# tongdaxu/VQ-VAE-from-Gaussian-VAE

Measured on AMD Instinct MI355X. Metric: images/sec encode+quantize+decode, 256x256, codebook 2^16, higher is better.
Workload: dtype f32

## Files before the change

### vq-vae-from-gaussian-vae_amd/csrc/gq_conv3.h

```cpp
#pragma once
#include <type_traits>

#include "gq_common.h"
#include "gq_epilogue.h"
#include "gq_stats.h"
#include "gq_wino_gemm.h"

namespace gqhip {

constexpr int kC3TH = 8, kC3TW = 32;
constexpr int kC3PH = kC3TH + 2, kC3PW = kC3TW + 2;
constexpr int kC3Pix = kC3PH * kC3PW;
constexpr int kC3RS = 48;
constexpr int kC3Plane = kC3PH * kC3RS * 32;
constexpr int kC3Buf = 2 * kC3Plane;
constexpr int kC3Pieces = kC3Pix * 4;
constexpr int kC3Loads = (kC3Pieces + 255) / 256;

__device__ __forceinline__ int conv3_lds_off(int R, int x, int half) {
  return (R * kC3RS + x) * 32 + 16 * (half ^ ((x >> 3) & 1));
}

struct Conv3Params {
  const _Float16 *Xs;
  const _Float16 *Wf;
  const float *bias;
  const float *res;
  float *y;
  int64_t *stats;
  int H, W, nch, cpg;
  int cout, nnb;
  int tiles_x, tiles_y;
  long ntiles;
  long tiles_per_xcd;
  float mscale;
};

struct Conv3Tile {
  long b;
  int y0, x0, nb;
};
__device__ __forceinline__ bool conv3_tile(const Conv3Params &p, Conv3Tile &t, long vb = blockIdx.x) {
  const long k = vb >> 3;
  t.nb = (int)(k % p.nnb);
  const long tile = (long)(vb & 7) * p.tiles_per_xcd + k / p.nnb;
  if (tile >= p.ntiles) return false;
  const int tx = (int)(tile % p.tiles_x);
  const long t2 = tile / p.tiles_x;
  t.b = t2 / p.tiles_y;
  t.y0 = (int)(t2 % p.tiles_y) * kC3TH;
  t.x0 = tx * kC3TW;
  return true;
}

__device__ __forceinline__ void conv3_tap(const unsigned char *A, int dy, const f16x8 (&bq)[4], f32x16 (&acc)[4][2]) {
#pragma unroll
  for (int rr = 0; rr < 4; ++rr) {
#if defined(GQHIP_ABL) && (GQHIP_ABL & 256)
    const f16x8 ah = *reinterpret_cast<const f16x8 *>(A + dy * kC3RS * 32);
    const f16x8 al = ah;
#else
    const f16x8 ah = *reinterpret_cast<const f16x8 *>(A + (rr + dy) * kC3RS * 32);
    const f16x8 al = *reinterpret_cast<const f16x8 *>(A + (rr + dy) * kC3RS * 32 + kC3Plane);
#endif
#pragma unroll
    for (int j = 0; j < 2; ++j) {
      acc[rr][j] = __builtin_amdgcn_mfma_f32_32x32x16_f16(ah, bq[2 * j], acc[rr][j], 0, 0, 0);
      acc[rr][j] = __builtin_amdgcn_mfma_f32_32x32x16_f16(ah, bq[2 * j + 1], acc[rr][j], 0, 0, 0);
      acc[rr][j] = __builtin_amdgcn_mfma_f32_32x32x16_f16(al, bq[2 * j], acc[rr][j], 0, 0, 0);
    }
  }
}

template <int COUT, int RR>
__device__ __forceinline__ void conv3_epilogue(const Conv3Params &p, const Conv3Tile &t, const f32x16 (&acc)[RR][2], unsigned char *sA,
                                               int64_t *red, int wave, int wm, int wn) {
  constexpr int cout = COUT;
  const int lane = __lane_id(), tid = wave * 64 + lane;
  const int n = wn * 64 + 4 * (lane & 15);
  float *stage = reinterpret_cast<float *>(sA + wave * kEpiWaveBytes);
  f32x4 pb = {0.f, 0.f, 0.f, 0.f};
  if (p.bias) {
#pragma unroll
    for (int e = 0; e < 4; ++e) pb[e] = p.bias[t.nb * 128 + n + e];
  }
  const long o = ((t.b * p.H + t.y0 + RR * wm) * p.W + t.x0 + (lane >> 4)) * cout + t.nb * 128 + n;
  const long slice = (long)p.W * cout;
  StatPartial st;
  if (!p.stats) {
    if (p.res) epi_store<3, false>(acc, stage, lane, p.y, p.res, o, slice, 4 * cout, p.mscale, pb, st);
    else epi_store<2, false>(acc, stage, lane, p.y, nullptr, o, slice, 4 * cout, p.mscale, pb, st);
    return;
  }
  if constexpr (RR == 4) {
    if (p.res) epi_store<3, true>(acc, stage, lane, p.y, p.res, o, slice, 4 * cout, p.mscale, pb, st);
    else epi_store<2, true>(acc, stage, lane, p.y, nullptr, o, slice, 4 * cout, p.mscale, pb, st);
    stat_partial_flush(red + kStatWords * (n / p.cpg), st);
  } else {
    __shared__ double part[2 * 64 * 4];
    double *mine = part + (wn * 64 + lane) * 4;
    if (wm == 0) {
      if (p.res) epi_store<3, true>(acc, stage, lane, p.y, p.res, o, slice, 4 * cout, p.mscale, pb, st);
      else epi_store<2, true>(acc, stage, lane, p.y, nullptr, o, slice, 4 * cout, p.mscale, pb, st);
      mine[0] = st.v0; mine[1] = st.s; mine[2] = st.ss; mine[3] = (double)st.n;
    }
    __syncthreads();
    if (wm == 1) {
      st.v0 = mine[0]; st.s = mine[1]; st.ss = mine[2]; st.n = (int)mine[3];
      if (p.res) epi_store<3, true>(acc, stage, lane, p.y, p.res, o, slice, 4 * cout, p.mscale, pb, st);
      else epi_store<2, true>(acc, stage, lane, p.y, nullptr, o, slice, 4 * cout, p.mscale, pb, st);
      stat_partial_flush(red + kStatWords * (n / p.cpg), st);
    }
  }
  __syncthreads();
  const int gpb = 128 / p.cpg, groups = cout / p.cpg;
  if (tid < kStatWords * gpb) stat_flush_word(p.stats + kStatWords * (t.b * groups + t.nb * gpb) + tid, red[tid]);
}

#define GQ_C3_ZERO_ACC(acc)                                                                                         \
  _Pragma("unroll") for (int rr = 0; rr < 4; ++rr) _Pragma("unroll") for (int j = 0; j < 2; ++j) acc[rr][j] =       \
      f32x16{0.f, 0.f, 0.f, 0.f, 0.f, 0.f, 0.f, 0.f, 0.f, 0.f, 0.f, 0.f, 0.f, 0.f, 0.f, 0.f}

struct Conv3GnParams {
  Conv3Params c;
  const float *x;
  const float *gamma, *beta, *pre_bias;
  const int64_t *stats_in;
  int cin, cpg_in;
  double eps;
  float scale;
};

#ifndef GQHIP_C3_VALU_PER_MFMA
#define GQHIP_C3_VALU_PER_MFMA 3
#endif
#ifdef GQHIP_CLOCK_STAMPS
__device__ unsigned long long g_c3_stamps[4 * 8192];
#endif
template <int SILU, int COUT>
__global__ __launch_bounds__(256, 2) void conv3x3_gn_f16x3_kernel(const Conv3GnParams pp) {
  typedef _Float16 f16x4 __attribute__((ext_vector_type(4)));
  const Conv3Params &p = pp.c;
  __shared__ __attribute__((aligned(16))) unsigned char sA[2 * kC3Buf];
  __shared__ int64_t red[kStatWords * 32];
  __shared__ __attribute__((aligned(16))) float sAff[2][512];
  const int tid = threadIdx.x, lane = tid & 63, wave = __builtin_amdgcn_readfirstlane(tid >> 6);
  const int c = lane & 31, h = lane >> 5, wm = wave >> 1, wn = wave & 1;
#ifdef GQHIP_CLOCK_STAMPS
  const unsigned long long st_r0 = __builtin_amdgcn_s_memrealtime();
#endif
  Conv3Tile t;
  if (!conv3_tile(p, t)) return;
  const int H = p.H, W = p.W, cin = pp.cin;
  red[tid] = 0;
  {
    const int groups = cin / pp.cpg_in;
    const double n = (double)pp.cpg_in * (double)H * (double)W;
    for (int ch = tid; ch < cin; ch += 256) {
      const GnAffine f = gn_channel(gn_group(pp.stats_in + kStatWords * (t.b * groups + ch / pp.cpg_in), n, pp.eps), pp.gamma, pp.beta, pp.pre_bias, ch);
      sAff[0][ch] = f.a;
      sAff[1][ch] = f.sh;
    }
  }
  const int w = tid & 3, qs = tid >> 2;
  int goff[kC3Loads];
  unsigned inb = 0;
#pragma unroll
  for (int i = 0; i < kC3Loads; ++i) {
    int q = qs + 64 * i;
    q = q < kC3Pix ? q : kC3Pix - 1;
    const int R = q / kC3PW, px = q % kC3PW;
    const int gy = t.y0 - 1 + R, gx = t.x0 - 1 + px;
    const bool in = gy >= 0 && gy < H && gx >= 0 && gx < W;
    const int cy = clamp_index(gy, H), cx = clamp_index(gx, W);
    goff[i] = (cy * W + cx) * cin + 4 * w;
    inb |= (unsigned)(in ? 1 : 0) << i;
  }
  const float *xb = pp.x + t.b * (long)H * W * cin;
  f32x4 st[3];
  auto issue = [&](int i, int chunk) { st[i % 3] = *reinterpret_cast<const f32x4 *>(xb + goff[i] + chunk * 16); };
  auto convert = [&](int i, int chunk, int buf) {
    const int q = qs + 64 * i < kC3Pix ? qs + 64 * i : kC3Pix - 1;
    const f32x4 a4 = *reinterpret_cast<const f32x4 *>(&sAff[0][chunk * 16 + 4 * w]);
    const f32x4 sh4 = *reinterpret_cast<const f32x4 *>(&sAff[1][chunk * 16 + 4 * w]);
    const f32x4 v = gn_act<SILU>(st[i % 3], a4, sh4) * (((inb >> i) & 1) ? pp.scale : 0.f);
    f16x4 hi, lo;
#pragma unroll
    for (int e = 0; e < 4; ++e) {
      hi[e] = (_Float16)v[e];
      lo[e] = (_Float16)(v[e] - (float)hi[e]);
    }
    const int off = buf * kC3Buf + conv3_lds_off(q / kC3PW, q % kC3PW, w >> 1) + 8 * (w & 1);
    *reinterpret_cast<f16x4 *>(&sA[off]) = hi;
    *reinterpret_cast<f16x4 *>(&sA[off + kC3Plane]) = lo;
  };

  f32x16 acc[4][2];
  GQ_C3_ZERO_ACC(acc);
  int aoff[3];
#pragma unroll
  for (int dx = 0; dx < 3; ++dx) aoff[dx] = conv3_lds_off(4 * wm, c + dx, h);
  const unsigned char *wbase = reinterpret_cast<const unsigned char *>(p.Wf) + (4 * t.nb + 2 * wn) * 128 * 16;
  const int wl = lane * 16;
  const long wstep = (long)p.nnb * (512 * 16);
  f16x8 bs[3][4];
  auto load_b = [&](int ks, f16x8 (&dst)[4]) {
    const unsigned char *s = wbase + ks * wstep;
#pragma unroll
    for (int k = 0; k < 4; ++k) dst[k] = *reinterpret_cast<const f16x8 *>(s + k * 1024 + wl);
  };
  const int nks = p.nch * 9;
  load_b(0, bs[0]);
  load_b(1, bs[1]);
  __syncthreads();
  for (int i0 = 0; i0 < kC3Loads; i0 += 3) {
#pragma unroll
    for (int i = 0; i < 3; ++i) issue(i0 + i, 0);
#pragma unroll
    for (int i = 0; i < 3; ++i) convert(i0 + i, 0, 0);
  }
  __syncthreads();

#ifdef GQHIP_CLOCK_STAMPS
  const unsigned long long st_r1 = __builtin_amdgcn_s_memrealtime();
#endif
  auto run_chunk = [&](int chunk, auto more_tag) {
    constexpr bool more = decltype(more_tag)::value;
    const unsigned char *A = sA + (chunk & 1) * kC3Buf;
    const int nbuf = (chunk + 1) & 1;
#pragma unroll
    for (int tap = 0; tap < 9; ++tap) {
      const int ks = chunk * 9 + tap;
#if !(defined(GQHIP_ABL) && (GQHIP_ABL & 128))
      load_b(ks + 2 < nks ? ks + 2 : nks - 1, bs[(tap + 2) % 3]);
#endif
      conv3_tap(A + aoff[tap % 3], tap / 3, bs[tap % 3], acc);
#if !(defined(GQHIP_ABL) && (GQHIP_ABL & 64))
      if constexpr (more) {
        if (tap >= 3) convert(tap - 3, chunk + 1, nbuf);
        if (tap < kC3Loads) issue(tap, chunk + 1);
#if GQHIP_C3_VALU_PER_MFMA > 0
        if (tap >= 3) {
#pragma unroll
          for (int m = 0; m < 24; ++m) {
            __builtin_amdgcn_sched_group_barrier(0x008, 1, 0);
            __builtin_amdgcn_sched_group_barrier(0x002, GQHIP_C3_VALU_PER_MFMA, 0);
          }
        }
#endif
      }
#endif
      __builtin_amdgcn_sched_barrier(0);
    }
    __syncthreads();
  };
  for (int chunk = 0; chunk + 1 < p.nch; ++chunk) run_chunk(chunk, std::true_type{});
  run_chunk(p.nch - 1, std::false_type{});
#ifdef GQHIP_CLOCK_STAMPS
  const unsigned long long st_r2 = __builtin_amdgcn_s_memrealtime();
#endif
#if defined(GQHIP_ABL) && (GQHIP_ABL & 512)
  if (acc[0][0][0] == 12345.678f)
#endif
  conv3_epilogue<COUT>(p, t, acc, sA, red, wave, wm, wn);
#ifdef GQHIP_CLOCK_STAMPS
  if (tid == 0 && blockIdx.x < 8192) {
    unsigned long long *o = g_c3_stamps + 4 * blockIdx.x;
    o[0] = st_r0;
    o[1] = __builtin_amdgcn_s_memrealtime();
    o[2] = ((st_r1 - st_r0) << 32) | (st_r2 - st_r0);
    o[3] = ((unsigned long long)__builtin_amdgcn_s_getreg((31 << 11) | 20) << 32) | (unsigned)__builtin_amdgcn_s_getreg((31 << 11) | 4);
  }
#endif
}



struct Conv1Params {
  Conv3Params c;
  const float *x;
  const float *pre_bias;
  const float *scales_dev;
  float scale;
  int cin;
  const float *gamma, *beta;
  const int64_t *stats_in;
  int cpg_in;
  double eps;
  _Float16 *Q3, *K3, *V3;
  float sq, sv;
};

template <int COUT, int RR, int GN, int SPLIT>
__global__ __launch_bounds__(256, 2) void conv1x1_f16x3_kernel(const Conv1Params pp) {
  typedef _Float16 f16x4 __attribute__((ext_vector_type(4)));
  static_assert(RR == 4 || RR == 2, "rows of 32 pixels per wave");
  static_assert((SPLIT != 0) == (COUT == 0), "the split epilogue takes cout at run time");
  Conv3Params p = pp.c;
  constexpr int NI = 2 * RR;
  constexpr int kPlane = 32 * NI * 32, kChunk = 2 * kPlane, kStage = 2 * kChunk;
  static_assert(2 * kStage >= 4 * kEpiWaveBytes, "the epilogue stages through sA");
  __shared__ __attribute__((aligned(16))) unsigned char sA[2 * kStage];
  __shared__ int64_t red[kStatWords * 32];
  __shared__ __attribute__((aligned(16))) float sAff[2][GN ? 512 : 4];
  const int tid = threadIdx.x, lane = tid & 63, wave = __builtin_amdgcn_readfirstlane(tid >> 6);
  const int c = lane & 31, h = lane >> 5, wm = wave >> 1, wn = wave & 1;
  Conv3Tile t;
  if (!conv3_tile(p, t)) return;
  t.y0 = t.y0 / kC3TH * NI;
  red[tid] = 0;
  const float scale = pp.scales_dev ? pp.scales_dev[0] : pp.scale;
  if (pp.scales_dev) p.mscale = pp.scales_dev[1];
  const int cin = pp.cin, nst = cin / 32;
  if constexpr (GN != 0) {
    const int groups = cin / pp.cpg_in;
    const double n = (double)pp.cpg_in * (double)p.H * 32.0;
    for (int ch = tid; ch < cin; ch += 256) {
      const GnAffine f = gn_channel(gn_group(pp.stats_in + kStatWords * (t.b * groups + ch / pp.cpg_in), n, pp.eps), pp.gamma, pp.beta, pp.pre_bias, ch);
      sAff[0][ch] = f.a;
      sAff[1][ch] = f.sh;
    }
  }
  const int w8 = tid & 7, r0 = tid >> 3;
  const float *xb = pp.x + ((t.b * p.H + t.y0) * 32L + r0) * cin + 4 * w8;
  const float *pbp = (GN == 0 && pp.pre_bias) ? pp.pre_bias + 4 * w8 : nullptr;
  f32x4 pb4 = {0.f, 0.f, 0.f, 0.f}, a4 = pb4, sh4 = pb4;
  const int loff = (w8 >> 2) * kChunk + r0 * 32 + 16 * (((w8 >> 1) & 1) ^ ((r0 >> 3) & 1)) + 8 * (w8 & 1);
  f32x4 st[NI];
  auto issue = [&](int stage) {
#pragma unroll
    for (int i = 0; i < NI; ++i) st[i] = *reinterpret_cast<const f32x4 *>(xb + (long)(32 * i) * cin + stage * 32);
  };
  auto affine = [&](int stage) {
    if constexpr (GN != 0) {
      a4 = *reinterpret_cast<const f32x4 *>(&sAff[0][stage * 32 + 4 * w8]);
      sh4 = *reinterpret_cast<const f32x4 *>(&sAff[1][stage * 32 + 4 * w8]);
    } else {
      if (pbp) pb4 = *reinterpret_cast<const f32x4 *>(pbp + stage * 32);
    }
  };
  auto convert = [&](int i, int buf) {
    f32x4 v;
    if constexpr (GN != 0) v = gn_act<0>(st[i], a4, sh4) * scale;
    else v = (st[i] + pb4) * scale;
    f16x4 hi, lo;
#pragma unroll
    for (int e = 0; e < 4; ++e) {
      hi[e] = (_Float16)v[e];
      lo[e] = (_Float16)(v[e] - (float)hi[e]);
    }
    unsigned char *d = sA + buf * kStage + loff + i * (32 * 32);
    *reinterpret_cast<f16x4 *>(d) = hi;
    *reinterpret_cast<f16x4 *>(d + kPlane) = lo;
  };
  f32x16 acc[RR][2];
#pragma unroll
  for (int rr = 0; rr < RR; ++rr)
#pragma unroll
    for (int j = 0; j < 2; ++j) acc[rr][j] = f32x16{0.f, 0.f, 0.f, 0.f, 0.f, 0.f, 0.f, 0.f, 0.f, 0.f, 0.f, 0.f, 0.f, 0.f, 0.f, 0.f};
  const int aoff = (RR * wm) * 1024 + c * 32 + 16 * (h ^ ((c >> 3) & 1));
  const unsigned char *wbase = reinterpret_cast<const unsigned char *>(p.Wf) + (4 * t.nb + 2 * wn) * 128 * 16;
  const int wl = lane * 16;
  const long wstep = (long)p.nnb * (512 * 16);
  f16x8 b0[4], b1[4];
  auto load_b = [&](int ks, f16x8 (&dst)[4]) {
    const unsigned char *s = wbase + ks * wstep;
#pragma unroll
    for (int k = 0; k < 4; ++k) dst[k] = *reinterpret_cast<const f16x8 *>(s + k * 1024 + wl);
  };
  auto kstep = [&](const unsigned char *A, const f16x8 (&bq)[4]) {
#pragma unroll
    for (int rr = 0; rr < RR; ++rr) {
      const f16x8 ah = *reinterpret_cast<const f16x8 *>(A + aoff + rr * 1024);
      const f16x8 al = *reinterpret_cast<const f16x8 *>(A + aoff + rr * 1024 + kPlane);
#pragma unroll
      for (int j = 0; j < 2; ++j) {
        acc[rr][j] = __builtin_amdgcn_mfma_f32_32x32x16_f16(ah, bq[2 * j], acc[rr][j], 0, 0, 0);
        acc[rr][j] = __builtin_amdgcn_mfma_f32_32x32x16_f16(ah, bq[2 * j + 1], acc[rr][j], 0, 0, 0);
        acc[rr][j] = __builtin_amdgcn_mfma_f32_32x32x16_f16(al, bq[2 * j], acc[rr][j], 0, 0, 0);
      }
    }
  };
  const int nks = 2 * nst;
  load_b(0, b0);
  issue(0);
  if constexpr (GN != 0) __syncthreads();
  affine(0);
#pragma unroll
  for (int i = 0; i < NI; ++i) convert(i, 0);
  __syncthreads();
  if constexpr (RR == 2) {
    auto run_stage = [&](int s, auto more_tag) {
      constexpr bool more = decltype(more_tag)::value;
      const unsigned char *A = sA + (s & 1) * kStage;
      const int nbuf = (s + 1) & 1;
      load_b(2 * s + 1, b1);
      if constexpr (more) issue(s + 1);
      kstep(A, b0);
      __builtin_amdgcn_sched_barrier(0);
      if constexpr (more) affine(s + 1);
      load_b(2 * s + 2 < nks ? 2 * s + 2 : nks - 1, b0);
      kstep(A + kChunk, b1);
      if constexpr (more) {
#pragma unroll
        for (int i = 0; i < NI; ++i) convert(i, nbuf);
#pragma unroll
        for (int m = 0; m < 6 * RR; ++m) {
          __builtin_amdgcn_sched_group_barrier(0x008, 1, 0);
          __builtin_amdgcn_sched_group_barrier(0x002, 8, 0);
        }
      }
      __builtin_amdgcn_sched_barrier(0);
      __syncthreads();
    };
    for (int s = 0; s + 1 < nst; ++s) run_stage(s, std::true_type{});
    run_stage(nst - 1, std::false_type{});
  } else {
    for (int s = 0; s < nst; ++s) {
      const bool more = s + 1 < nst;
      const unsigned char *A = sA + (s & 1) * kStage;
      const int nbuf = (s + 1) & 1;
      load_b(2 * s + 1, b1);
      if (more) issue(s + 1);
      kstep(A, b0);
      __builtin_amdgcn_sched_barrier(0);
      load_b(2 * s + 2 < nks ? 2 * s + 2 : nks - 1, b0);
      kstep(A + kChunk, b1);
      if (more) {
        affine(s + 1);
#pragma unroll
        for (int i = 0; i < NI; ++i) convert(i, nbuf);
      }
      __builtin_amdgcn_sched_barrier(0);
      __syncthreads();
    }
  }
  if constexpr (SPLIT != 0) {
    const int C = p.cout / 3, col = t.nb * 128, third = col / C;
    const int n = wn * 64 + 4 * (lane & 15), cc = col - third * C + n;
    const long L = (long)p.H * 32, tok = (long)(t.y0 + RR * wm) * 32 + (lane >> 4);
    f32x4 pb = {0.f, 0.f, 0.f, 0.f};
    if (p.bias) {
#pragma unroll
      for (int e = 0; e < 4; ++e) pb[e] = p.bias[col + n + e];
    }
    float *stage = reinterpret_cast<float *>(sA + wave * kEpiWaveBytes);
    if (third < 2) {
      _Float16 *dst = third == 0 ? pp.Q3 : pp.K3;
      epi_store_split(acc, stage, lane, dst, (t.b * L + tok) * 3 * C + cc, 32L * 3 * C, 4L * 3 * C, (long)C, third == 0, p.mscale,
                      pb, pp.sq);
    } else {
      epi_store_split(acc, stage, lane, pp.V3, (t.b * 3 * L + tok) * C + cc, 32L * C, 4L * C, L * C, false, p.mscale, pb, pp.sv);
    }
  } else {
    conv3_epilogue<COUT>(p, t, acc, sA, red, wave, wm, wn);
  }
}

struct Conv3S2Params {
  Conv3Params c;
  const float *x;
  const float *scales_dev;
  float scale;
  int cin, Hin, Win;
};

template <int COUT>
__global__ __launch_bounds__(256, 2) void conv3x3s2_f16x3_kernel(const Conv3S2Params pp) {
  typedef _Float16 f16x4 __attribute__((ext_vector_type(4)));
  Conv3Params p = pp.c;
  __shared__ __attribute__((aligned(16))) unsigned char sA[2 * kC3Buf];
  __shared__ int64_t red[kStatWords * 32];
  const int tid = threadIdx.x, lane = tid & 63, wave = __builtin_amdgcn_readfirstlane(tid >> 6);
  const int c = lane & 31, h = lane >> 5, wm = wave >> 1, wn = wave & 1;
  Conv3Tile t;
  if (!conv3_tile(p, t)) return;
  red[tid] = 0;
  const float scale = pp.scales_dev ? pp.scales_dev[0] : pp.scale;
  if (pp.scales_dev) p.mscale = pp.scales_dev[1];
  const int cin = pp.cin, nch = p.nch, Hin = pp.Hin, Win = pp.Win;
  constexpr int PR = kC3TH + 1, PC = kC3TW + 1, NP = 5;
  const int w = tid & 3, qs = tid >> 2;
  const float *xb = pp.x + t.b * (long)Hin * Win * cin + 4 * w;
  int goff[NP], loff[NP];
  unsigned inb = 0;
  auto setup_phase = [&](int a, int b) {
    inb = 0;
#pragma unroll
    for (int i = 0; i < NP; ++i) {
      const int q = qs + 64 * i;
      const int qq = q < PR * PC ? q : PR * PC - 1;
      const int R = qq / PC, X = qq % PC;
      const int gy = 2 * (t.y0 + R) + a, gx = 2 * (t.x0 + X) + b;
      const bool in = gy < Hin && gx < Win;
      const int cy = gy < Hin ? gy : Hin - 1, cx = gx < Win ? gx : Win - 1;
      goff[i] = (cy * Win + cx) * cin;
      loff[i] = q < PR * PC ? conv3_lds_off(R, X, w >> 1) + 8 * (w & 1) : -1;
      inb |= (unsigned)(in ? 1 : 0) << i;
    }
  };
  f32x4 st[NP];
  auto issue = [&](int chunk) {
#pragma unroll
    for (int i = 0; i < NP; ++i) st[i] = *reinterpret_cast<const f32x4 *>(xb + goff[i] + chunk * 16);
  };
  auto commit = [&](int buf) {
#pragma unroll
    for (int i = 0; i < NP; ++i) {
      if (loff[i] < 0) continue;
      const f32x4 v = st[i] * (((inb >> i) & 1) ? scale : 0.f);
      f16x4 hi, lo;
#pragma unroll
      for (int e = 0; e < 4; ++e) {
        hi[e] = (_Float16)v[e];
        lo[e] = (_Float16)(v[e] - (float)hi[e]);
      }
      unsigned char *d = sA + buf * kC3Buf + loff[i];
      *reinterpret_cast<f16x4 *>(d) = hi;
      *reinterpret_cast<f16x4 *>(d + kC3Plane) = lo;
    }
  };
  f32x16 acc[4][2];
  GQ_C3_ZERO_ACC(acc);
  int aoff[2];
#pragma unroll
  for (int dx = 0; dx < 2; ++dx) aoff[dx] = conv3_lds_off(4 * wm, c + dx, h);
  const unsigned char *wbase = reinterpret_cast<const unsigned char *>(p.Wf) + (4 * t.nb + 2 * wn) * 128 * 16;
  const int wl = lane * 16;
  const long wstep = (long)p.nnb * (512 * 16);
  f16x8 bq[4], bn[4];
  auto load_b = [&](int ks, f16x8 (&dst)[4]) {
    const unsigned char *s = wbase + ks * wstep;
#pragma unroll
    for (int k = 0; k < 4; ++k) dst[k] = *reinterpret_cast<const f16x8 *>(s + k * 1024 + wl);
  };
  const int nks = 9 * nch;
  int ks = 0, unit = 0;
  load_b(0, bq);
  setup_phase(0, 0);
  issue(0);
  commit(0);
  __syncthreads();
  auto run_unit = [&](auto nt_tag, auto a_tag, auto b_tag, int chunk) {
    constexpr int NT = decltype(nt_tag)::value, PA = decltype(a_tag)::value, PB = decltype(b_tag)::value;
    const bool last_chunk = chunk + 1 >= nch;
    const bool more = !(last_chunk && PA == 1 && PB == 1);
    if (more) {
      if (last_chunk) setup_phase(PB == 1 ? 1 : PA, PB == 1 ? 0 : 1);
      issue(last_chunk ? 0 : chunk + 1);
    }
    const unsigned char *A = sA + (unit & 1) * kC3Buf;
#pragma unroll
    for (int ti = 0; ti < NT; ++ti) {
      const int ddy = (PA == 0 && PB == 0) ? ti / 2 : (PA == 0 && PB == 1) ? ti : 0;
      const int ddx = (PA == 0 && PB == 0) ? ti % 2 : (PA == 1 && PB == 0) ? ti : 0;
      load_b(ks + 1 < nks ? ks + 1 : ks, bn);
      conv3_tap(A + aoff[ddx], ddy, bq, acc);
#pragma unroll
      for (int k = 0; k < 4; ++k) bq[k] = bn[k];
      ++ks;
      __builtin_amdgcn_sched_barrier(0);
    }
    if (more) commit((unit + 1) & 1);
    ++unit;
    __syncthreads();
  };
  using I0 = std::integral_constant<int, 0>; using I1 = std::integral_constant<int, 1>;
  using I2 = std::integral_constant<int, 2>; using I4 = std::integral_constant<int, 4>;
  for (int chunk = 0; chunk < nch; ++chunk) run_unit(I4{}, I0{}, I0{}, chunk);
  for (int chunk = 0; chunk < nch; ++chunk) run_unit(I2{}, I0{}, I1{}, chunk);
  for (int chunk = 0; chunk < nch; ++chunk) run_unit(I2{}, I1{}, I0{}, chunk);
  for (int chunk = 0; chunk < nch; ++chunk) run_unit(I1{}, I1{}, I1{}, chunk);
  conv3_epilogue<COUT>(p, t, acc, sA, red, wave, wm, wn);
}

struct Upconv2Params {
  Conv3Params c;
  const float *x;
  const float *scales_dev;
  float scale;
  int cin;
};

template <int COUT>
__global__ __launch_bounds__(256, 2) void upconv2x_f16x3_kernel(const Upconv2Params pp) {
  typedef _Float16 f16x4 __attribute__((ext_vector_type(4)));
  Conv3Params p = pp.c;
  __shared__ __attribute__((aligned(16))) unsigned char sA[2 * kC3Buf];
  __shared__ int64_t red[kStatWords * 32];
  const int tid = threadIdx.x, lane = tid & 63, wave = __builtin_amdgcn_readfirstlane(tid >> 6);
  const int c = lane & 31, h = lane >> 5, wm = wave >> 1, wn = wave & 1;
  Conv3Tile t;
  if (!conv3_tile(p, t)) return;
  const int pa = (int)blockIdx.y >> 1, pb = (int)blockIdx.y & 1;
  red[tid] = 0;
  const float scale = pp.scales_dev ? pp.scales_dev[0] : pp.scale;
  if (pp.scales_dev) p.mscale = pp.scales_dev[1];
  const int cin = pp.cin, nch = p.nch, H = p.H, W = p.W;
  constexpr int PR = kC3TH + 1, PC = kC3TW + 1, NP = 5;
  const int w = tid & 3, qs = tid >> 2;
  const float *xb = pp.x + t.b * (long)H * W * cin + 4 * w;
  int goff[NP], loff[NP];
  unsigned inb = 0;
#pragma unroll
  for (int i = 0; i < NP; ++i) {
    const int q = qs + 64 * i;
    const int qq = q < PR * PC ? q : PR * PC - 1;
    const int R = qq / PC, X = qq % PC;
    const int gy = t.y0 + R + pa - 1, gx = t.x0 + X + pb - 1;
    const bool in = gy >= 0 && gy < H && gx >= 0 && gx < W;
    const int cy = gy < 0 ? 0 : (gy >= H ? H - 1 : gy), cx = gx < 0 ? 0 : (gx >= W ? W - 1 : gx);
    goff[i] = (cy * W + cx) * cin;
    loff[i] = conv3_lds_off(R, X, w >> 1) + 8 * (w & 1);
    inb |= (unsigned)(in ? 1 : 0) << i;
  }
  f32x4 st[NP];
  auto issue = [&](int chunk) {
#pragma unroll
    for (int i = 0; i < NP; ++i) st[i] = *reinterpret_cast<const f32x4 *>(xb + goff[i] + chunk * 16);
  };
  auto commit_piece = [&](int i, int buf) {
    const f32x4 v = st[i] * (((inb >> i) & 1) ? scale : 0.f);
    f16x4 hi, lo;
#pragma unroll
    for (int e = 0; e < 4; ++e) {
      hi[e] = (_Float16)v[e];
      lo[e] = (_Float16)(v[e] - (float)hi[e]);
    }
    unsigned char *d = sA + buf * kC3Buf + loff[i];
    *reinterpret_cast<f16x4 *>(d) = hi;
    *reinterpret_cast<f16x4 *>(d + kC3Plane) = lo;
  };
  f32x16 acc[4][2];
  GQ_C3_ZERO_ACC(acc);
  int aoff[2];
#pragma unroll
  for (int dx = 0; dx < 2; ++dx) aoff[dx] = conv3_lds_off(4 * wm, c + dx, h);
  const long wstep = (long)p.nnb * (512 * 16);
  const int nks = 4 * nch;
  const unsigned char *wbase = reinterpret_cast<const unsigned char *>(p.Wf) + (long)blockIdx.y * nks * wstep +
                               (4 * t.nb + 2 * wn) * 128 * 16;
  const int wl = lane * 16;
  f16x8 b0[4], b1[4], b2[4];
  auto load_b = [&](int ks, f16x8 (&dst)[4]) {
    const unsigned char *s = wbase + (long)(ks < nks ? ks : nks - 1) * wstep;
#pragma unroll
    for (int k = 0; k < 4; ++k) dst[k] = *reinterpret_cast<const f16x8 *>(s + k * 1024 + wl);
  };
  load_b(0, b0);
  load_b(1, b1);
  issue(0);
#pragma unroll
  for (int i = 0; i < NP; ++i) commit_piece(i, 0);
  __syncthreads();
  int ks = 0;
  auto run_chunk = [&](int chunk, auto more_tag) {
    constexpr bool more = decltype(more_tag)::value;
    if constexpr (more) issue(chunk + 1);
    const unsigned char *A = sA + (chunk & 1) * kC3Buf;
    const int nbuf = (chunk + 1) & 1;
#pragma unroll
    for (int ti = 0; ti < 4; ++ti) {
      load_b(ks + 2, b2);
      conv3_tap(A + aoff[ti & 1], ti >> 1, b0, acc);
#pragma unroll
      for (int k = 0; k < 4; ++k) {
        b0[k] = b1[k];
        b1[k] = b2[k];
      }
      ++ks;
      if constexpr (more) {
        if (ti == 2) {
          commit_piece(0, nbuf);
          commit_piece(1, nbuf);
        }
        if (ti == 3) {
          commit_piece(2, nbuf);
          commit_piece(3, nbuf);
          commit_piece(4, nbuf);
        }
        if (ti >= 2) {
#pragma unroll
          for (int m = 0; m < 24; ++m) {
            __builtin_amdgcn_sched_group_barrier(0x008, 1, 0);
            __builtin_amdgcn_sched_group_barrier(0x002, 3, 0);
          }
        }
      }
      __builtin_amdgcn_sched_barrier(0);
    }
    __syncthreads();
  };
  for (int chunk = 0; chunk + 1 < nch; ++chunk) run_chunk(chunk, std::true_type{});
  run_chunk(nch - 1, std::false_type{});
  constexpr int cout = COUT;
  const int n = wn * 64 + 4 * (lane & 15);
  f32x4 bias4 = {0.f, 0.f, 0.f, 0.f};
  if (p.bias) {
#pragma unroll
    for (int e = 0; e < 4; ++e) bias4[e] = p.bias[t.nb * 128 + n + e];
  }
  float *stage = reinterpret_cast<float *>(sA + wave * kEpiWaveBytes);
  const long W2 = 2L * W;
  const long o = ((t.b * 2L * H + 2 * (t.y0 + 4 * wm) + pa) * W2 + 2 * (t.x0 + (lane >> 4)) + pb) * cout + t.nb * 128 + n;
  StatPartial sp;
  if (!p.stats) {
    epi_store<1, false>(acc, stage, lane, p.y, nullptr, o, 2 * W2 * cout, 8 * cout, p.mscale, bias4, sp);
    return;
  }
  epi_store<1, true>(acc, stage, lane, p.y, nullptr, o, 2 * W2 * cout, 8 * cout, p.mscale, bias4, sp);
  stat_partial_flush(red + kStatWords * (n / p.cpg), sp);
  __syncthreads();
  const int gpb = 128 / p.cpg, groups = cout / p.cpg;
  if (tid < kStatWords * gpb) stat_flush_word(p.stats + kStatWords * (t.b * groups + t.nb * gpb) + tid, red[tid]);
}

template <int SILU, int COUT>
__global__ __launch_bounds__(256) void conv3x3_gn_small_kernel(const float *__restrict__ x, const float *__restrict__ gamma,
                                                               const float *__restrict__ beta,
                                                               const float *__restrict__ pre_bias,
                                                               const int64_t *__restrict__ stats, const float *__restrict__ w,
                                                               const float *__restrict__ bias, float *__restrict__ y, int H,
                                                               int W, int C, int cpg, double eps) {
  constexpr int PW = 18, PS = 36;
  __shared__ __attribute__((aligned(16))) float sX[PW * PW * PS];
  __shared__ __attribute__((aligned(16))) float sAff[2][512];
  const int tid = threadIdx.x, tx = tid & 15, ty = tid >> 4;
  const int tiles_x = W / 16, tiles_y = H / 16;
  const int txb = blockIdx.x % tiles_x, tyb = (blockIdx.x / tiles_x) % tiles_y;
  const long b = blockIdx.x / (tiles_x * tiles_y);
  const int y0 = tyb * 16, x0 = txb * 16;
  {
    const int groups = C / cpg;
    const double n = (double)cpg * (double)H * (double)W;
    for (int ch = tid; ch < C; ch += 256) {
      const GnAffine f = gn_channel(gn_group(stats + kStatWords * (b * groups + ch / cpg), n, eps), gamma, beta, pre_bias, ch);
      sAff[0][ch] = f.a;
      sAff[1][ch] = f.sh;
    }
  }
  float acc[COUT];
#pragma unroll
  for (int co = 0; co < COUT; ++co) acc[co] = bias ? bias[co] : 0.f;
  const float *xb = x + b * (long)H * W * C;
  __syncthreads();
  for (int c0 = 0; c0 < C; c0 += 32) {
    for (int i = tid; i < PW * PW * 8; i += 256) {
      const int px = i >> 3, q = i & 7;
      const int R = px / PW, X = px % PW;
      const int gy = y0 - 1 + R, gx = x0 - 1 + X;
      const bool in = gy >= 0 && gy < H && gx >= 0 && gx < W;
      const int cy = clamp_index(gy, H), cx = clamp_index(gx, W);
      const f32x4 v = *reinterpret_cast<const f32x4 *>(xb + ((long)cy * W + cx) * C + c0 + 4 * q);
      const f32x4 a4 = *reinterpret_cast<const f32x4 *>(&sAff[0][c0 + 4 * q]);
      const f32x4 sh4 = *reinterpret_cast<const f32x4 *>(&sAff[1][c0 + 4 * q]);
      *reinterpret_cast<f32x4 *>(&sX[px * PS + 4 * q]) = gn_act<SILU>(v, a4, sh4) * (in ? 1.f : 0.f);
    }
    __syncthreads();
#pragma unroll
    for (int tap = 0; tap < 9; ++tap) {
      const float *s = &sX[((ty + tap / 3) * PW + tx + tap % 3) * PS];
#pragma unroll
      for (int q = 0; q < 8; ++q) {
        const f32x4 v = *reinterpret_cast<const f32x4 *>(s + 4 * q);
#pragma unroll
        for (int co = 0; co < COUT; ++co) {
          const float *wp = w + ((long)(co * 9 + tap) * C + c0 + 4 * q);
          acc[co] = __builtin_fmaf(v.x, wp[0], acc[co]);
          acc[co] = __builtin_fmaf(v.y, wp[1], acc[co]);
          acc[co] = __builtin_fmaf(v.z, wp[2], acc[co]);
          acc[co] = __builtin_fmaf(v.w, wp[3], acc[co]);
        }
      }
    }
    __syncthreads();
  }
  float *yo = y + ((b * H + y0 + ty) * W + x0 + tx) * COUT;
#pragma unroll
  for (int co = 0; co < COUT; ++co) yo[co] = acc[co];
}

}
```

Measured before the change: 520.3.

## Prefetch next channel chunk into registers during small GN conv3x3 compute

Restructures the small-output GN+conv3x3 kernel so the global loads for the next 32-channel chunk are issued into registers before the tap loop. They are converted with the GN affine and activation and written to LDS only after compute finishes, overlapping load latency with FMAs. The tile fill is also remapped to a fixed per-thread row/column layout with a few extra edge loads, and a scheduling barrier is added inside the tap loop. This costs more registers (eleven float4 staged per thread) and disables unrolling of the tap loop, which could cut occupancy or ILP.

New measurement: 522.0 (median of 6 runs). About the same (+0.3%).

```diff
diff --git a/vq-vae-from-gaussian-vae_amd/csrc/gq_conv3.h b/vq-vae-from-gaussian-vae_amd/csrc/gq_conv3.h
--- a/vq-vae-from-gaussian-vae_amd/csrc/gq_conv3.h
+++ b/vq-vae-from-gaussian-vae_amd/csrc/gq_conv3.h
@@ -723,6 +723,7 @@
                                                                const float *__restrict__ bias, float *__restrict__ y, int H,
                                                                int W, int C, int cpg, double eps) {
   constexpr int PW = 18, PS = 36;
+  constexpr int NQM = PW / 2, NQE = 2, NQ = NQM + NQE;
   __shared__ __attribute__((aligned(16))) float sX[PW * PW * PS];
   __shared__ __attribute__((aligned(16))) float sAff[2][512];
   const int tid = threadIdx.x, tx = tid & 15, ty = tid >> 4;
@@ -743,21 +744,55 @@
 #pragma unroll
   for (int co = 0; co < COUT; ++co) acc[co] = bias ? bias[co] : 0.f;
   const float *xb = x + b * (long)H * W * C;
+  const int q8 = tid & 7, sc = (tid >> 3) & 15, sr = tid >> 7;
+  const bool sc_in = x0 - 1 + sc >= 0;
+  const int xoff = clamp_index(x0 - 1 + sc, W) * C + 4 * q8;
+  f32x4 st[NQ];
+  auto extra = [&](int j, int &R, int &X) {
+    const int px = min((tid >> 3) + 32 * j, 2 * PW - 1);
+    R = px >> 1;
+    X = 16 + (px & 1);
+  };
+  auto issue = [&](int c0) {
+#pragma unroll
+    for (int i = 0; i < NQM; ++i) {
+      const int cy = clamp_index(y0 - 1 + 2 * i + sr, H);
+      st[i] = *reinterpret_cast<const f32x4 *>(xb + (long)cy * W * C + c0 + xoff);
+    }
+#pragma unroll
+    for (int j = 0; j < NQE; ++j) {
+      int R, X;
+      extra(j, R, X);
+      const int cy = clamp_index(y0 - 1 + R, H), cx = clamp_index(x0 - 1 + X, W);
+      st[NQM + j] = *reinterpret_cast<const f32x4 *>(xb + ((long)cy * W + cx) * C + c0 + 4 * q8);
+    }
+  };
+  auto convert = [&](int c0) {
+    const f32x4 a4 = *reinterpret_cast<const f32x4 *>(&sAff[0][c0 + 4 * q8]);
+    const f32x4 sh4 = *reinterpret_cast<const f32x4 *>(&sAff[1][c0 + 4 * q8]);
+#pragma unroll
+    for (int i = 0; i < NQM; ++i) {
+      const int R = 2 * i + sr, gy = y0 - 1 + R;
+      const bool in = gy >= 0 && gy < H && sc_in;
+      *reinterpret_cast<f32x4 *>(&sX[(R * PW + sc) * PS + 4 * q8]) = gn_act<SILU>(st[i], a4, sh4) * (in ? 1.f : 0.f);
+    }
+#pragma unroll
+    for (int j = 0; j < NQE; ++j) {
+      int R, X;
+      extra(j, R, X);
+      const int gy = y0 - 1 + R, gx = x0 - 1 + X;
+      const bool in = gy >= 0 && gy < H && gx < W;
+      *reinterpret_cast<f32x4 *>(&sX[(R * PW + X) * PS + 4 * q8]) = gn_act<SILU>(st[NQM + j], a4, sh4) * (in ? 1.f : 0.f);
+    }
+  };
+  issue(0);
+  __syncthreads();
+  convert(0);
   __syncthreads();
   for (int c0 = 0; c0 < C; c0 += 32) {
-    for (int i = tid; i < PW * PW * 8; i += 256) {
-      const int px = i >> 3, q = i & 7;
-      const int R = px / PW, X = px % PW;
-      const int gy = y0 - 1 + R, gx = x0 - 1 + X;
-      const bool in = gy >= 0 && gy < H && gx >= 0 && gx < W;
-      const int cy = clamp_index(gy, H), cx = clamp_index(gx, W);
-      const f32x4 v = *reinterpret_cast<const f32x4 *>(xb + ((long)cy * W + cx) * C + c0 + 4 * q);
-      const f32x4 a4 = *reinterpret_cast<const f32x4 *>(&sAff[0][c0 + 4 * q]);
-      const f32x4 sh4 = *reinterpret_cast<const f32x4 *>(&sAff[1][c0 + 4 * q]);
-      *reinterpret_cast<f32x4 *>(&sX[px * PS + 4 * q]) = gn_act<SILU>(v, a4, sh4) * (in ? 1.f : 0.f);
-    }
-    __syncthreads();
-#pragma unroll
+    const bool more = c0 + 32 < C;
+    if (more) issue(c0 + 32);
+#pragma unroll 1
     for (int tap = 0; tap < 9; ++tap) {
       const float *s = &sX[((ty + tap / 3) * PW + tx + tap % 3) * PS];
 #pragma unroll
@@ -771,9 +806,14 @@
           acc[co] = __builtin_fmaf(v.z, wp[2], acc[co]);
           acc[co] = __builtin_fmaf(v.w, wp[3], acc[co]);
         }
+        if (COUT >= 3 && q == 3) __builtin_amdgcn_sched_barrier(0);
       }
     }
     __syncthreads();
+    if (more) {
+      convert(c0 + 32);
+      __syncthreads();
+    }
   }
   float *yo = y + ((b * H + y0 + ty) * W + x0 + tx) * COUT;
 #pragma unroll
```
